# ISAE-PNX/SaDVIO

Measured on AMD Instinct MI355X. Metric: BA iterations/sec (ms/solve in ms_per_solve), 20-KF/8k-landmark window, higher is better.
Workload: dtype f64; 1 GPU; synthetic 20 KF x 8000 landmarks x 40000 reprojection factors (pixel), GN 10 iters (LM step attempts, early exits disabled); windows_per_gpu=1, parallelism=single window, n_kf=20, n_lmk=8000, n_obs=40000, reduced_dim=114

## Files before the change

### sadvio_amd/csrc/ba_capi.hip

```cpp
#include <hip/hip_runtime.h>
#include <dlfcn.h>

#include <algorithm>
#include <chrono>
#include <cmath>
#include <cstdio>
#include <cstdlib>
#include <cstring>
#include <map>
#include <string>
#include <vector>

#include "../../include/sadvio_ba.h"
#include "kernels.h"
#include "dense_chol.h"
#include "marg_kernels.h"
#include "lm_kernels.h"
#include "viinit_kernels.h"
#include "nofov_kernels.h"

using namespace sadvio;

namespace {

// ... 161 lines not shown
struct TriLevel { int first, count, max_m, max_n; };
struct MargScratch {
    DevBuf<double> A, b, G, V, ev, Vs, Ainv, T, Ak, bk, newJ, newr, lastJ, lastr, L, Tb, Zt, S, mi, jsel, lam, wtmp, Hl;
    DevBuf<int> ditems, flag, sel, lastcol, piv_of, lc, piv_mm;
    DevBuf<MargSmall> small;
    DevBuf<NfrSpecC> spec;
    std::vector<int> lcol, items, items_l, col;
    std::vector<double> hev, hS;
    struct TriPlan { DevBuf<TriNode> nodes; std::vector<TriLevel> levels; int leaves = 0; };
    std::map<int, TriPlan> tri_plans;
};

struct LineSetHost {
    std::vector<int64_t> id;
    std::vector<double> T, model, meas;
    std::vector<unsigned char> is_const;
    std::vector<int> ptr, obs_kf, obs_cam;
    int n() const { return (int)id.size(); }
};

struct LayoutScratch {
    std::vector<double> kf_T0, kf_vel, kf_ba, kf_bg, cam_K, cam_T, cam_isig, lmk_p, obs_meas;
    std::vector<int> kf_fidx, lmk_ob, lmk_oe, obs_kf, obs_cam, tile_kf, tile_row, pkf, pcam, run_max, idx, mark, add, kfs, slot_of, chunk_ob, chunk_lm, perm;
    std::vector<unsigned char> lmk_const, obs_slot, obs_lslot;
    std::vector<char> held;
};

struct EnvCfg {
    int debug = 0;
    int lm = -1, pf_wg = -1;
    int tile_rounds = 0, lm_subs = 0, band_c = 0;
    double jacobi_tol = 1e-14;
    bool marg_last_small = false, marg_eig_mm = false, marg_pivoted = false, marg_unpivoted = false, pchol_swap = false, pchol_strict = false,
         jacobi_b4 = false, jacobi_plain = false, no_lpt = false, no_pre = false, no_fork = false, no_bcr = false, imu_items = false;
    void read() {
        auto on = [](const char* k) { return getenv(k) != nullptr; };
        auto num = [](const char* k, int unset) { const char* e = getenv(k); return e ? atoi(e) : unset; };
        debug = num("SADVIO_DEBUG", 0); lm = num("SADVIO_LM", -1); pf_wg = num("SADVIO_PF_WG", -1);
        tile_rounds = num("SADVIO_TILE_ROUNDS", 0); lm_subs = num("SADVIO_LM_SUBS", 0); band_c = num("SADVIO_BAND_C", 0);
        if (const char* e = getenv("SADVIO_JACOBI_TOL")) jacobi_tol = atof(e);
        marg_last_small = on("SADVIO_MARG_LAST_SMALL"); marg_eig_mm = on("SADVIO_MARG_EIG_MM"); marg_pivoted = on("SADVIO_MARG_PIVOTED");
        marg_unpivoted = on("SADVIO_MARG_UNPIVOTED"); pchol_swap = on("SADVIO_PCHOL_SWAP"); pchol_strict = on("SADVIO_PCHOL_STRICT");
        jacobi_b4 = on("SADVIO_JACOBI_B4"); jacobi_plain = on("SADVIO_JACOBI_PLAIN"); no_lpt = on("SADVIO_NO_LPT"); no_pre = on("SADVIO_NO_PRE"); no_fork = on("SADVIO_NO_FORK");
        no_bcr = on("SADVIO_NO_BCR");
        imu_items = on("SADVIO_IMU_ITEMS");
    }
};

struct sadvio_ba_handle {
    EnvCfg env;
    sadvio_ba_config cfg{};
    LayoutScratch ls;
    int device = 0;
    hipStream_t stream = nullptr;
    std::string err;
    std::vector<HostWin> wins;
    std::vector<Tile> tiles;
    std::vector<PriorDev> priors;
    std::vector<int> obs_perm;
    std::vector<std::vector<PriorDev>> priors_per_win;
    std::vector<std::vector<ImuDev>> imus_per_win;
    std::vector<ImuDev> imus;
    int n_kf_tot = 0, n_cam_tot = 0, n_lmk_tot = 0, n_obs_tot = 0, np_tot = 0;
    long long s_tot = 0;
    int factor_type = 0;
    int max_n_kf = 0, max_npose = 0, max_np = 0, n_big = 0;
    DevBuf<int> d_big_info;
    DevBuf<double> d_big_M;
    DevBuf<double> d_big_Lx;
    DevBuf<double> d_big_linv;
    DevBuf<double> d_coll_band;
    DevBuf<double> d_bcr;
    DevBuf<double> d_big_mid;
    bool uploaded = false, solved = false;
    bool defer = false, pending = false;
    UploadBatch up;
// ... 8 lines not shown
    MargScratch mg;
    std::vector<SrcWin> src;
    std::vector<std::vector<char>> sp_elim;
    std::vector<int> n_obs_user;
    std::vector<std::vector<sadvio_sparse_prior>> sparse_per_win;
    std::vector<LineSetHost> lines_per_win;
    DevBuf<LineDev> d_lines;
    DevBuf<LineObsDev> d_lobs;
    DevBuf<double> d_xline, d_line_scratch;
    int n_line_tot = 0, n_lobs_tot = 0;
    DevBuf<SparseDev> d_sparse;
    DevBuf<int> d_sp_list;
    int n_sp_list = 0;
    size_t n_sparse_tot = 0;
    DevBuf<double> d_sp_scratch;
    std::vector<unsigned char> h_lmk_const_user;
    std::vector<int> h_lmk_ob, h_lmk_oe, h_kf_fidx, h_obs_kf;
    bool user_lmk_const = false;
    int n_kept = 0;
    DevBuf<int> d_lmk_red, d_kept_obs, d_dp_ints;
    DevBuf<double> d_dp_data;
    int slots_cap = 0;
    int last_slots = 0;
    DevBuf<WinDev> d_win;
    DevBuf<Tile> d_tiles;
    DevBuf<double> d_kf_T0, d_xp, d_xv, d_xba, d_xbg, d_kf_vel, d_kf_ba, d_kf_bg;
    DevBuf<int> d_kf_fidx;
    DevBuf<double> d_cam_K, d_cam_T, d_cam_isig;
    DevBuf<double> d_lmk_p, d_xl, d_s_lmk;
    DevBuf<unsigned char> d_lmk_const;
    DevBuf<int> d_lmk_ob, d_lmk_oe, d_obs_kf, d_obs_cam, d_tile_kf, d_tile_row;
    DevBuf<int> d_pre_lane, d_pre_kf;
    bool pre_ok = false, pre_dirty = false;
    DevBuf<int> d_rank_col; DevBuf<double> d_rank_x;
    DevBuf<unsigned char> d_obs_slot, d_obs_lslot;
    DevBuf<int> d_chunk_ob, d_chunk_lm, d_tile_perm;
    DevBuf<int> d_jac_ints;
    DevBuf<double> d_jac_dbl;
    DevBuf<double> d_lm_hg, d_lm_dt, d_lm_sacc;
    DevBuf<int> d_lm_sub;
    int lm_n_sub = 0, lm_ksub = 1, lm_sub_per_item = 8;
    int lm_max_cam = 1;
    int hidden_eig_count = 0;
    int marg_stats[4] = {0, 0, 0, 0};
    int lm_sub_obs = 0;
    bool gemm_run4 = false;
    bool lm_ok = false;
    long long lm_landmarks = 0;
    DevBuf<double> d_ptab;
    int max_tile_kf = 1, max_tile_free = 0, max_gemm_free = 0;
    DevBuf<double> d_obs_meas;
    DevBuf<PriorDev> d_priors;
    DevBuf<double> d_prior_lin;
    DevBuf<ImuDev> d_imus;
    DevBuf<double> d_imu_scratch;
    DevBuf<double> d_S, d_gred, d_gfull, d_hdiag, d_delta, d_s_pose;
    DevBuf<LmState> d_states;
    DevBuf<double> d_trace;
    DevBuf<long long> d_tstart;
    DevBuf<IterAcc> d_acc;
    DevBuf<FinalRec> d_final;
    FinalRec* h_final = nullptr;
    double* h_deltas = nullptr; size_t h_deltas_cap = 0; bool deltas_cached = false;
    size_t h_final_n = 0;
    std::vector<FinalRec> fin;
    DevBuf<TileAcc> d_tacc;
// ... 35 lines not shown
        (void)hipEventRecord(h->ev_pool[pool].first, h->stream);
    }
    ~ScopedTimer() {
        if (pool >= 0) (void)hipEventRecord(h->ev_pool[pool].second, h->stream);
    }
};

void collect_timers(sadvio_ba_handle* h) {
    for (auto& u : h->ev_used) {
        float ms = 0;
        if (hipEventElapsedTime(&ms, h->ev_pool[u.second].first, h->ev_pool[u.second].second) == hipSuccess) {
            h->kclasses[u.first].total_ms += ms;
            h->kclasses[u.first].launches += 1;
        }
    }
    h->ev_used.clear();
    h->ev_next = 0;
}

DevPtrs make_ptrs(sadvio_ba_handle* h, const SolveOpts& o, int state_stride) {
    DevPtrs P{};
    P.win = h->d_win.p; P.tiles = h->d_tiles.p;
    P.kf_T0 = h->d_kf_T0.p; P.kf_fidx = h->d_kf_fidx.p;
    P.xp = h->d_xp.p; P.xv = h->d_xv.p; P.xba = h->d_xba.p; P.xbg = h->d_xbg.p;
    P.xp_stride = 6LL * h->n_kf_tot; P.xv_stride = 3LL * h->n_kf_tot; P.xl_stride = 3LL * h->n_lmk_tot;
    P.kf_vel = h->d_kf_vel.p; P.kf_ba = h->d_kf_ba.p; P.kf_bg = h->d_kf_bg.p;
    P.cam_K = h->d_cam_K.p; P.cam_T = h->d_cam_T.p; P.cam_isig = h->d_cam_isig.p;
    P.lmk_p = h->d_lmk_p.p; P.xl = h->d_xl.p; P.s_lmk = h->d_s_lmk.p;
    P.lmk_const = h->has_lmk_const ? h->d_lmk_const.p : nullptr;
    P.lmk_ob = h->d_lmk_ob.p; P.lmk_oe = h->d_lmk_oe.p;
    P.obs_kf = h->d_obs_kf.p; P.obs_cam = h->d_obs_cam.p; P.obs_meas = h->d_obs_meas.p;
    P.obs_slot = h->d_obs_slot.p; P.tile_kf = h->d_tile_kf.p; P.tile_row = h->d_tile_row.p;
    P.pre_lane = h->pre_ok ? (const int4*)h->d_pre_lane.p : nullptr; P.pre_kf = h->pre_ok ? (const int2*)h->d_pre_kf.p : nullptr;
    P.ptab = h->d_ptab.p; P.ptab_stride = (long long)POSE_TAB * h->n_kf_tot;
    P.priors = h->d_priors.p; P.prior_lin = h->d_prior_lin.p; P.prior_lin_stride = (long long)h->priors.size() * PRIOR_LIN; P.n_prior_tot = (int)h->priors.size();
    P.imus = h->d_imus.p; P.imu_scratch = h->d_imu_scratch.p; P.imu_scratch_stride = (long long)h->imus.size() * IMU_ROW;
    P.S = h->d_S.p; P.gred = h->d_gred.p; P.gfull = h->d_gfull.p; P.hdiag = h->d_hdiag.p;
    P.delta = h->d_delta.p; P.s_pose = h->d_s_pose.p;
    P.dbg_ts = h->d_dbg.p;
    P.trace = h->d_trace.p; P.t_start = h->d_tstart.p;
    P.states = h->d_states.p; P.acc = h->d_acc.p; P.tacc = h->d_tacc.p; P.n_tiles = (int)h->tiles.size();
    P.state_stride = state_stride;
    P.final_out = h->h_final ? h->h_final : h->d_final.p;
    P.big_info = h->d_big_info.p;
    P.world = h->world; P.rank = h->rank; P.rank_b = h->d_rank_b.p; P.rank_s = h->d_rank_s.p;
    P.lmk_red = h->d_lmk_red.p; P.kept_obs = h->d_kept_obs.p; P.n_kept = h->n_kept;
    P.dp_data = h->d_dp_data.p; P.dp_ints = h->d_dp_ints.p;
    P.sparse = h->d_sparse.p; P.sp_scratch = h->d_sp_scratch.p; P.sp_list = h->d_sp_list.p;
    P.sp_scratch_stride = (long long)std::max<size_t>(h->n_sparse_tot, 1) * SPARSE_J; P.n_imu_tot = (int)h->imus.size(); P.n_sp_list = h->n_sp_list;
    P.chunk_ob = h->d_chunk_ob.p; P.chunk_lm = h->d_chunk_lm.p; P.tile_perm = h->d_tile_perm.p; P.obs_lslot = h->d_obs_lslot.p;
    P.lm_hg = h->d_lm_hg.p; P.lm_hg_stride = (long long)LM_HG * std::max(h->n_lmk_tot, 1);
    P.lm_dt = h->d_lm_dt.p; P.lm_dt_stride = (long long)LM_DT * std::max<long long>((long long)h->tiles.size(), 1) * h->lm_ksub;
    P.lm_sub = h->d_lm_sub.p; P.lm_ksub = h->lm_ksub; P.lm_sub_per_item = h->lm_sub_per_item; P.lm_sacc = h->lm_ok ? h->d_lm_sacc.p : nullptr;
    P.lines = h->d_lines.p; P.lobs = h->d_lobs.p; P.xline = h->d_xline.p; P.line_scratch = h->d_line_scratch.p;
    P.xline_stride = 6LL * h->n_line_tot;
    P.n_xp = (long long)h->d_xp.n; P.n_xv = (long long)h->d_xv.n; P.n_xl = (long long)h->d_xl.n;
    P.n_win = (int)h->wins.size();
    P.debug = h->env.debug;
    P.o = o;
    return P;
}

__global__ void k_dense_prior_prepare(const double* J, double* Jt, int nf, int n) {
    const long long idx = (long long)blockIdx.x * blockDim.x + threadIdx.x;
    if (idx < (long long)nf * n) {
        const int i = (int)(idx / n), a = (int)(idx - (long long)i * n);
// ... 705 lines not shown
        h->up.add(h->d_lm_sub.p, sub.data(), sub.size() * sizeof(int));
    }
    if (h->env.debug) {
        int hist[32] = {0}, modes[3] = {0};
        for (auto& t : h->tiles) { hist[std::min(t.n_free, 31)]++; modes[t.lds_mode]++; }
        fprintf(stderr, "[sadvio dbg] %zu tiles, modes global/atomic/gemm = %d/%d/%d, max_tile_kf %d, n_free histogram:", h->tiles.size(), modes[0], modes[1], modes[2], h->max_tile_kf);
        for (int i = 0; i < 32; i++) if (hist[i]) fprintf(stderr, " %d:%d", i, hist[i]);
        fprintf(stderr, "\n");
    }
    HIP_TRY(h->d_win.alloc(n_windows)); HIP_TRY(h->d_tacc.alloc(2 * h->tiles.size()));
    if (tile_kf.empty()) { tile_kf.push_back(0); tile_row.push_back(-1); }
    HIP_TRY(h->d_tile_kf.alloc(tile_kf.size())); HIP_TRY(h->d_tile_row.alloc(tile_row.size()));
    HIP_TRY(h->d_obs_slot.alloc(obs_slot.size())); HIP_TRY(h->d_ptab.alloc(2 * (size_t)POSE_TAB * kf_b));
    HIP_TRY(h->d_kf_T0.alloc(kf_T0.size())); HIP_TRY(h->d_kf_fidx.alloc(kf_fidx.size()));
    HIP_TRY(h->d_xp.alloc(2 * 6 * (size_t)kf_b)); HIP_TRY(h->d_xv.alloc(2 * 3 * (size_t)kf_b));
    HIP_TRY(h->d_xba.alloc(2 * 3 * (size_t)kf_b)); HIP_TRY(h->d_xbg.alloc(2 * 3 * (size_t)kf_b));
    HIP_TRY(h->d_kf_vel.alloc(kf_vel.size())); HIP_TRY(h->d_kf_ba.alloc(kf_ba.size())); HIP_TRY(h->d_kf_bg.alloc(kf_bg.size()));
    HIP_TRY(h->d_cam_K.alloc(cam_K.size())); HIP_TRY(h->d_cam_T.alloc(cam_T.size())); HIP_TRY(h->d_cam_isig.alloc(cam_isig.size()));
    HIP_TRY(h->d_lmk_p.alloc(lmk_p.size())); HIP_TRY(h->d_xl.alloc(2 * 3 * (size_t)std::max(lmk_b, 1)));
    HIP_TRY(h->d_s_lmk.alloc(3 * (size_t)std::max(lmk_b, 1)));
    HIP_TRY(h->d_lmk_ob.alloc(lmk_ob.size())); HIP_TRY(h->d_lmk_oe.alloc(lmk_oe.size()));
    HIP_TRY(h->d_obs_kf.alloc(obs_kf.size())); HIP_TRY(h->d_obs_cam.alloc(obs_cam.size())); HIP_TRY(h->d_obs_meas.alloc(obs_meas.size()));
#define UP(dst, src) h->up.add((dst).p, (src).data(), (src).size() * sizeof((src)[0]))
    UP(h->d_kf_T0, kf_T0); UP(h->d_kf_fidx, kf_fidx); UP(h->d_kf_vel, kf_vel);
    UP(h->d_kf_ba, kf_ba); UP(h->d_kf_bg, kf_bg); UP(h->d_cam_K, cam_K); UP(h->d_cam_T, cam_T); UP(h->d_cam_isig, cam_isig);
    if (lmk_b) { UP(h->d_lmk_p, lmk_p); }
    UP(h->d_lmk_ob, lmk_ob); UP(h->d_lmk_oe, lmk_oe); UP(h->d_obs_kf, obs_kf);
    UP(h->d_obs_cam, obs_cam); UP(h->d_obs_meas, obs_meas); UP(h->d_tile_kf, tile_kf); UP(h->d_tile_row, tile_row); UP(h->d_obs_slot, obs_slot);
    h->pre_ok = !h->tiles.empty() && h->tiles.size() <= PRE_MAX_TILES && !h->env.no_pre;
    if (h->pre_ok) {
        HIP_TRY(h->d_pre_lane.alloc((size_t)4 * (BUILD_THREADS / 8) * h->tiles.size())); HIP_TRY(h->d_pre_kf.alloc((size_t)2 * PRE_KF * h->tiles.size()));
        h->pre_dirty = true;
    }
#undef UP
    h->h_lmk_const_user = lmk_const; h->user_lmk_const = h->has_lmk_const;
    h->h_lmk_ob = lmk_ob; h->h_lmk_oe = lmk_oe; h->h_kf_fidx = kf_fidx; h->h_obs_kf = obs_kf;
    lap("alloc+queue");
    int rc = layout_reduced(h);
    if (rc != SADVIO_OK) return rc;
    lap("layout_reduced");
    rc = upload_priors(h);
    if (rc != SADVIO_OK) return rc;
    lap("flush");
    h->uploaded = true;
    for (auto& k : h->kclasses) { k.total_ms = 0; k.launches = 0; }
    return SADVIO_OK;
}

int sadvio_ba_set_windows(sadvio_ba_handle* h, int32_t n_windows, const sadvio_flat_window* wins) {
    if (!h) return SADVIO_E_INVALID_ARG;
    if (n_windows <= 0 || !wins) { h->err = "set_windows: no windows"; return SADVIO_E_INVALID_ARG; }
    h->uploaded = false; h->solved = false;
    for (int w = 0; w < n_windows; w++) {
        const sadvio_flat_window& F = wins[w];
        if (F.n_kf <= 0 || F.n_cam < 0 || F.n_lmk < 0 || F.n_obs < 0 || !F.kf_T_f_w || (F.n_cam > 0 && (!F.cam_K || !F.cam_T_s_f)) ||
            (F.n_obs > 0 && F.n_cam == 0) ||
            (F.n_lmk > 0 && (!F.lmk_p || !F.lmk_obs_ptr)) || (F.n_obs > 0 && (!F.obs_kf || !F.obs_cam || !F.obs_meas))) {
            h->err = "set_windows: missing array in window " + std::to_string(w);
            return SADVIO_E_INVALID_ARG;
        }
        if (F.n_lmk > 0 && (F.lmk_obs_ptr[0] != 0 || F.lmk_obs_ptr[F.n_lmk] != F.n_obs)) {
            h->err = "set_windows: lmk_obs_ptr is not a CSR over n_obs";
            return SADVIO_E_INVALID_ARG;
        }
        for (int l = 0; l < F.n_lmk; l++)
            if (F.lmk_obs_ptr[l + 1] < F.lmk_obs_ptr[l]) { h->err = "set_windows: CSR not monotone"; return SADVIO_E_INVALID_ARG; }
// ... 1517 lines not shown
        h->max_gemm_free = 0;
        Rp = 0; strip_doubles = STAGE_VALS * 64;
        lds_build = tile_tables_bytes(mtk) + sizeof(double) * ((size_t)BUILD_WAVES * strip_doubles + nt * (nt + 1) / 2 + 3 * nt +
                                                               0) + 16;
    }
    if (h->env.debug) fprintf(stderr, "[sadvio dbg] lds_build %zu B, Rp %d, strip_doubles %d, max_tile_kf %d, max_tile_free %d, tiles %d\n", lds_build, Rp, strip_doubles, mtk, h->max_tile_free, n_tiles);
    const size_t lds_back = tile_tables_bytes(mtk) + sizeof(double) * ((size_t)mtk * 18) + 16;
    const size_t npq = (size_t)h->max_np;
    const size_t lds_solve = sizeof(double) * ((size_t)c16_size((int)npq) + 4 * npq + 1 + C16_WORK + 16 * (size_t)c16_blocks((int)npq + 1) + SOLVE_KFC * SOLVE_KFC_STRIDE) + 64;
    bool any_pseudo = false;
    for (const auto& v : h->sp_elim) for (char e : v) any_pseudo |= e != 0;
    bool any_kept_lmk = false;
    for (int w = 0; w < n_win; w++) any_kept_lmk |= h->wins[w].d.n_red > 0;
    const bool rare = o.huber_a > 0.0 || h->n_kept > 0 || any_kept_lmk || any_pseudo || h->gemm_run4;
    const bool pix = h->factor_type == SADVIO_FACTOR_PIXEL;
    const bool have_pf = !h->imus.empty() || h->n_sp_list > 0;
    bool with_imu = have_pf && n_tiles <= 3 * 256;
    if (h->env.pf_wg >= 0) with_imu = have_pf && h->env.pf_wg != 0;
    auto kb = with_imu ? (pix ? (rare ? k_build<0, true, true> : k_build<0, false, true>) : (rare ? k_build<1, true, true> : k_build<1, false, true>))
                       : (pix ? (rare ? k_build<0, true, false> : k_build<0, false, false>) : (rare ? k_build<1, true, false> : k_build<1, false, false>));
    auto kk = with_imu ? (pix ? (rare ? k_backsub<0, true, true> : k_backsub<0, false, true>) : (rare ? k_backsub<1, true, true> : k_backsub<1, false, true>))
                       : (pix ? (rare ? k_backsub<0, true, false> : k_backsub<0, false, false>) : (rare ? k_backsub<1, true, false> : k_backsub<1, false, false>));
    auto kbk = h->factor_type == SADVIO_FACTOR_PIXEL ? k_build_kept<0> : k_build_kept<1>;
    bool use_lm = h->lm_ok && !rare && !h->coll_fn && h->world == 1 && h->lm_landmarks >= 65536;
    if (h->env.lm >= 0) use_lm = h->lm_ok && !rare && !h->coll_fn && h->world == 1 && h->env.lm != 0;
    auto kbo = pix ? k_build_obs<0> : k_build_obs<1>;
    auto kps = pix ? k_lm_pass<0, false> : k_lm_pass<1, false>;
    auto kps0 = pix ? k_lm_pass<0, true> : k_lm_pass<1, true>;
    const size_t lds_views = pix ? sizeof(double) * (size_t)mtk * h->lm_max_cam * LM_VT : 0;
    const size_t lds_bobs = tile_tables_bytes(mtk) + sizeof(double) * ((size_t)BUILD_WAVES * Rp * LM_KS + nt * (nt + 1) / 2 + nt + 1 + LM_DT) + lds_views + 16;
    const size_t lds_pass0 = tile_tables_bytes(mtk) + sizeof(double) * LM_DT_COST + (size_t)h->lm_sub_obs * ((pix ? 2 : 3) * sizeof(double) + sizeof(int)) + lds_views + 16;
    const size_t lds_pass = lds_pass0 + sizeof(double) * (size_t)mtk * (POSE_TAB + 6) + lds_views;
    if (!use_lm) P.lm_sacc = nullptr;
    if (use_lm) {
        P.decide_kernel = 1;
        HIP_TRY(hipFuncSetAttribute((const void*)kbo, hipFuncAttributeMaxDynamicSharedMemorySize, (int)lds_bobs));
        HIP_TRY(hipFuncSetAttribute((const void*)kps, hipFuncAttributeMaxDynamicSharedMemorySize, (int)lds_pass));
        HIP_TRY(hipFuncSetAttribute((const void*)kps0, hipFuncAttributeMaxDynamicSharedMemorySize, (int)lds_pass0));
    }
    HIP_TRY(hipFuncSetAttribute((const void*)kb, hipFuncAttributeMaxDynamicSharedMemorySize, (int)lds_build));
    HIP_TRY(hipFuncSetAttribute((const void*)kk, hipFuncAttributeMaxDynamicSharedMemorySize, (int)lds_back));
    bool extras = false;
    for (int w = 0; w < n_win; w++) {
        const WinDev& d = h->wins[w].d;
        if (d.imu_end > d.imu_begin || d.sp_end > d.sp_begin || d.dp_n_full > 0 || d.dpf == 15 || d.lobs_end > d.lobs_begin || d.line_end > d.line_begin) extras = true;
    }
    auto ks0 = extras ? k_solve<0, true> : k_solve<0, false>;
    auto ks1 = extras ? k_solve<1, true> : k_solve<1, false>;
    auto ks2 = extras ? k_solve<2, true> : k_solve<2, false>;
    HIP_TRY(hipFuncSetAttribute((const void*)ks0, hipFuncAttributeMaxDynamicSharedMemorySize, (int)lds_solve));
    const int reset_blocks = (int)std::min<long long>(1024, std::max<long long>(1, (P.n_xl + P.n_xp + 255) / 256));
    std::vector<BigPlan> big(n_win);
    for (int w = 0; w < n_win; w++) {
        const WinDev& d = h->wins[w].d;
        if (!d.ld) continue;
        int hb = h->wins[w].hb_lmk;
        for (const ImuDev& f : h->imus_per_win[w]) {
            const int fi = h->h_kf_fidx[f.kf_i], fj = h->h_kf_fidx[f.kf_j];
            if (fi >= 0 && fj >= 0) hb = std::max(hb, std::abs(fi - fj));
        }
        if (w < (int)h->sparse_per_win.size())
            for (const sadvio_sparse_prior& sp : h->sparse_per_win[w])
                if (sp.type == SADVIO_SPARSE_RELATIVE_POSE) {
                    const int fi = h->h_kf_fidx[d.kf_base + sp.kf], fj = h->h_kf_fidx[d.kf_base + sp.kf_b];
                    if (fi >= 0 && fj >= 0) hb = std::max(hb, std::abs(fi - fj));
                }
// ... 103 lines not shown
            if (fork) {
                (void)hipEventRecord(h->ev_solved, h->stream);
                (void)hipStreamWaitEvent(h->side, h->ev_solved, 0);
                if (n_lo) hipLaunchKernelGGL(k_line_eval<false>, dim3(n_lo), dim3(64), 0, h->side, P, s, 0);
                (void)hipEventRecord(h->ev_cost, h->side);
            } else {
                if (n_lo) { ScopedTimer t(h, "k_line_cost"); hipLaunchKernelGGL(k_line_eval<false>, dim3(n_lo), dim3(64), 0, h->stream, P, s, 0); }
            }
            if (dp_max_nf > 0) { ScopedTimer t(h, "k_prior_m"); hipLaunchKernelGGL(k_prior_m, dim3((dp_max_nf + 3) / 4, n_win), dim3(256), 0, h->stream, P, s); }
            if (n_pf && (use_lm || !with_imu)) { ScopedTimer t(h, "k_pf_cost"); hipLaunchKernelGGL(k_pf_eval<true>, dim3(n_pf), dim3(64), 0, h->stream, P, s); }
            if (use_lm) {
                ScopedTimer t(h, "k_lm_pass"); hipLaunchKernelGGL(kps, dim3(h->lm_n_sub), dim3(LM_PASS_THREADS), lds_pass, h->stream, P, s, mtk, h->lm_sub_obs);
            }
            else
            { ScopedTimer t(h, "k_backsub"); hipLaunchKernelGGL(kk, dim3(n_tiles + (with_imu ? n_pf : 0)), dim3(BUILD_THREADS), lds_back, h->stream, P, s, mtk); }
            if (fork) (void)hipStreamWaitEvent(h->stream, h->ev_cost, 0);
            if (h->coll_fn) {
                { ScopedTimer t(h, "k_rank_partials"); hipLaunchKernelGGL(k_rank_partials, dim3(n_win), dim3(64), 0, h->stream, P, s, 1); }
                ScopedTimer t(h, "allreduce_step_partials");
                if (h->coll_fn(h->coll_ctx, h->d_rank_s.p, (int64_t)n_win * h->world * 4, (void*)h->stream) != 0) coll_failed = true;
            }
            if (P.decide_kernel) { ScopedTimer t(h, "k_decide"); hipLaunchKernelGGL(k_decide, dim3(n_win), dim3(max_win_tiles > 4 * BUILD_THREADS ? 1024 : 64), 0, h->stream, P, s, 0); }
        }
        { ScopedTimer t(h, "k_final"); hipLaunchKernelGGL(k_decide, dim3(n_win), dim3(64), 0, h->stream, P, slots - 1, 1); }
    };
    if (h->cfg.use_graph && !h->cfg.profile_kernels && !h->coll_fn) {
        std::vector<int> lay;
        for (int w = 0; w < n_win; w++) { lay.push_back(h->wins[w].d.Np); lay.push_back(h->wins[w].d.ld); lay.push_back(big[w].bw); }
        lay.push_back(h->n_kept); lay.push_back(h->lm_sub_obs); lay.push_back(h->lm_n_sub); lay.push_back(h->lm_max_cam); lay.push_back(h->n_lobs_tot); lay.push_back(h->n_line_tot); lay.push_back(h->n_big); lay.push_back(dp_max_nf); lay.push_back(dp_max_n);
        std::vector<unsigned char> key(sizeof(DevPtrs) + 8 * sizeof(int) + 3 * sizeof(size_t) + lay.size() * sizeof(int));
        unsigned char* kp = key.data();
        memcpy(kp + sizeof(DevPtrs) + 8 * sizeof(int) + 3 * sizeof(size_t), lay.data(), lay.size() * sizeof(int));
        memcpy(kp, &P, sizeof(DevPtrs)); kp += sizeof(DevPtrs);
        const int env_bits = (int)with_imu + 2 * (int)h->env.no_fork + 32 * (int)h->env.no_bcr + 128 * (int)h->env.no_lpt;
        const int ints[8] = {slots, n_tiles, n_win, mtk, strip_doubles, Rp, h->n_kf_tot, h->factor_type + 2 * (int)extras + 4 * (int)rare + 8 * (int)use_lm + 16 * env_bits};
        memcpy(kp, ints, sizeof(ints)); kp += sizeof(ints);
        const size_t szs[3] = {lds_build, lds_back, lds_solve};
        memcpy(kp, szs, sizeof(szs));
        if (!h->graph_exec || key != h->graph_key) {
            if (h->graph_exec) { (void)hipGraphExecDestroy(h->graph_exec); h->graph_exec = nullptr; }
            hipGraph_t g = nullptr;
            HIP_TRY(hipStreamBeginCapture(h->stream, hipStreamCaptureModeThreadLocal));
            enqueue();
            HIP_TRY(hipStreamEndCapture(h->stream, &g));
            HIP_TRY(hipGraphInstantiate(&h->graph_exec, g, nullptr, nullptr, 0));
            (void)hipGraphDestroy(g);
            h->graph_key = key;
        }
        HIP_TRY(hipGraphLaunch(h->graph_exec, h->stream));
    } else {
        enqueue();
    }
    HIP_TRY(hipGetLastError());
    if (coll_failed) { h->err = "solve: the all-reduce of the reduced system failed"; return SADVIO_E_RCCL; }
    HIP_TRY(hipStreamSynchronize(h->stream));
    if (h->cfg.profile_kernels) collect_timers(h);
    if ((h->env.debug & 4096)) {
        long long ts[128];
        if (hipMemcpy(ts, h->d_dbg.p, sizeof(ts), hipMemcpyDeviceToHost) == hipSuccess) {
            fprintf(stderr, "[sadvio dbg] phase dt (us):");
            for (int i = 1; i < 16; i++) fprintf(stderr, " %d:%.2f", i, (ts[i] - ts[0]) * 0.01);
            fprintf(stderr, "  shader clock %.3f GHz\n[sadvio dbg] k_build:", (double)(ts[21] - ts[20]) / ((ts[15] - ts[0]) * 10.0));
            for (int i = 33; i < 43; i++) fprintf(stderr, " %d:%.2f", i, (ts[i] - ts[32]) * 0.01);
            fprintf(stderr, "\n[sadvio dbg] first IMU pair of k_build, us since its start (residual + Jacobian on lane 0 | decision | W J | entries + adds): %.2f %.2f %.2f %.2f, start %.2f us after tile 0",
                    (ts[57] - ts[56]) * 0.01, (ts[58] - ts[56]) * 0.01, (ts[59] - ts[56]) * 0.01, (ts[60] - ts[56]) * 0.01, (ts[56] - ts[32]) * 0.01);
            fprintf(stderr, "\n[sadvio dbg] k_wchol_step (panel 1), us since the workgroup's start: look-ahead (operands in LDS | substituted | block updated | factored) %.2f %.2f %.2f %.2f",
                    (ts[107] - ts[106]) * 0.01, (ts[108] - ts[106]) * 0.01, (ts[109] - ts[106]) * 0.01, (ts[110] - ts[106]) * 0.01);
// ... 394 lines not shown
```

### sadvio_amd/csrc/ba_types.h

```cpp
#pragma once
#include <stdint.h>

namespace sadvio {

struct SolveOpts {
    int max_num_iterations;
    int jacobi_scaling;
    int max_num_consecutive_invalid_steps;
    int pad;
    double function_tolerance, gradient_tolerance, parameter_tolerance;
    double initial_radius, max_radius, min_radius;
    double min_lm_diagonal, max_lm_diagonal, min_relative_decrease;
    double huber_a;
    double max_time_ticks;
};

struct WinDev {
    int n_kf, n_cam, n_lmk, n_obs;
    int kf_base, cam_base, lmk_base, obs_base;
    int n_free_kf, dpf, Np, Npose;
    long long S_off;
    int red_off;
    int tile_begin, tile_end;
    int prior_begin, prior_end;
// ... 88 lines not shown

struct IterAcc {
    double lin_cost;
    double cand_cost;
    double mcc;
    double step_norm2;
    double cand_norm2;
    double fixed_cost;
    unsigned long long gmax_bits;
    int chol_fail;
    int time_up;
};

struct TileAcc {
    double lin_cost, fixed_cost, gmax;
    double cand_cost, mcc, step_norm2, cand_norm2;
    double pad;
};

constexpr int BUILD_THREADS = 256;
constexpr int BUILD_WAVES = BUILD_THREADS / 64;
constexpr int MAX_TILE_KF = 24;
constexpr int MAX_TILE_FREE_KF = 20;
constexpr int MAX_GEMM_FREE_KF = 5;
constexpr int MAX_WIN_CAM = 8;
constexpr int STAGE_VALS = 18;
constexpr int MAX_LMK_OBS = 64;
constexpr int SOLVE_THREADS = 512;
constexpr int SOLVE_KFC_STRIDE = 32;
constexpr int SOLVE_KFC = 32;
constexpr int PRIOR_LIN = 28;
constexpr int PRE_KF = 8;
constexpr int PRE_MAX_TILES = 1024;
constexpr int MAX_LDS_NP = 174;

}
```

### sadvio_amd/csrc/kernels.h

```cpp
#pragma once
#include "ba_types.h"
#include "device_math.h"
#include "chol16.h"

namespace sadvio {

struct DevPtrs {
    const WinDev* win;
    const Tile* tiles;
    const double* kf_T0;
    const int* kf_fidx;
    double* xp; double* xv; double* xba; double* xbg;
    long long xp_stride, xv_stride, xl_stride;
    const double* kf_vel; const double* kf_ba; const double* kf_bg;
    const double* cam_K; const double* cam_T; const double* cam_isig;
    const double* lmk_p; double* xl; double* s_lmk;
    const unsigned char* lmk_const;
    const int* lmk_ob; const int* lmk_oe;
    const int* obs_kf; const int* obs_cam; const double* obs_meas;
    const unsigned char* obs_slot;
    const int* tile_kf;
    const int* tile_row;
    const int4* pre_lane;
    const int2* pre_kf;
    double* ptab;
    long long ptab_stride;
    const PriorDev* priors;
    double* prior_lin;
    long long prior_lin_stride;
    int n_prior_tot;
    const ImuDev* imus;
    double* imu_scratch;
    long long imu_scratch_stride;
    double* S; double* gred; double* gfull; double* hdiag; double* delta; double* s_pose;
    LmState* states;
    IterAcc* acc;
    TileAcc* tacc;
    FinalRec* final_out;
    int* big_info;
    int imu_direct;
    int decide_kernel;
    int world, rank;
    double* rank_b;
    double* rank_s;
    const int* lmk_red;
    const int* kept_obs;
    int n_kept;
    double* dp_data;
    const SparseDev* sparse;
    const int* sp_list;
    double* sp_scratch;
    long long sp_scratch_stride;
    int n_imu_tot, n_sp_list;
    const int* dp_ints;
    const int* chunk_ob;
    const int* chunk_lm;
    const int* tile_perm;
// ... 544 lines not shown
        const int nobs = lmk_valid ? oe - ob : 0;
        const int lcode = first ? pre_lcode : (P.lmk_const ? P.lmk_const[gl] : 0);
        const bool lfree = lcode == 0;
        ObsLin L;
        L.valid = q < nobs;
        L.row = -1; L.slot = 0; L.counted = false;
        if (L.valid) {
            double pw[3];
            ObsPre obq;
            if (first) {
#pragma unroll
                for (int i = 0; i < 3; i++) pw[i] = pre_p[i] + (st.cur ? pre_x1[i] : pre_x0[i]);
                obq = pre_obs;
            } else {
#pragma unroll
                for (int i = 0; i < 3; i++) pw[i] = P.lmk_p[3 * (long long)gl + i] + xl[3 * (long long)gl + i];
                obq = obs_prefetch<FACTOR>(P, ob + q);
            }
            lane_linearize<FACTOR, RARE>(P, poseTab, camTab, rowTab, T.cam_base, obq, pw, lfree, lcode != 1, L);
            const double c = L.rho;
            if (L.counted) cost_part += c;
            else { fixed_part += c; L.r[0] = 0.0; L.r[1] = 0.0; }
        } else {
            L.r[0] = L.r[1] = 0.0;
#pragma unroll
            for (int i = 0; i < 12; i++) L.Jp[i] = 0.0;
#pragma unroll
            for (int i = 0; i < 6; i++) L.Jl[i] = 0.0;
        }
    SADVIO_TS(3, 35);
        double Mi[6], g[3];
        const bool active = group_eliminate(P, L, G, gl, lmk_valid, lfree, nobs, st.radius, slot == 0, q == 0, Mi, g);
        if (active && q == 0) gmax_part = fmax(gmax_part, fmax(fabs(g[0]), fmax(fabs(g[1]), fabs(g[2]))));
    SADVIO_TS(3, 36);
        double N[6], gam[3];
        li_row(Mi, L.Jl[0], L.Jl[1], L.Jl[2], N);
        li_row(Mi, L.Jl[3], L.Jl[4], L.Jl[5], N + 3);
        li_vec(Mi, g, gam);
        if (gemm_mode) {
            constexpr int Kw = 32, KS = Kw + 2;
            double* Yb = wstage;
            const double* Eb = Yb;
            {
                double2* z = (double2*)wstage;
                const double2 zero2 = make_double2(0.0, 0.0);
                for (int i = ln; i < Rp * KS / 2; i += 64) z[i] = zero2;
            }
            const bool vrow = L.valid && L.row >= 0;
            const int myrow = vrow ? L.row : -2 - ln;
            const int row_prev = dpp_i32<0x111>(myrow);
            const int row_next = dpp_i32<0x101>(myrow);
            const bool follower = vrow && q > 0 && row_prev == myrow;
            const bool has_follower = vrow && q + 1 < G && row_next == myrow;
            const int row_next2 = RARE ? dpp_i32<0x102>(myrow) : -1;
            const bool has_follower2 = RARE && vrow && q + 2 < G && row_next2 == myrow;
            const bool head = vrow && !follower;
            const double rt0 = L.r[0] - (N[0] * gam[0] + N[1] * gam[1] + N[2] * gam[2]);
            const double rt1 = L.r[1] - (N[3] * gam[0] + N[4] * gam[1] + N[5] * gam[2]);
            wave_lds_fence();
    SADVIO_TS(3, 37);
#pragma unroll
            for (int i = 0; i < 6; i++) {
                const double j0 = vrow ? L.Jp[i] : 0.0, j1 = vrow ? L.Jp[6 + i] : 0.0;
                double y[3];
#pragma unroll
                for (int c = 0; c < 3; c++) {
// ... 1105 lines not shown
        acc->step_norm2 = a0; acc->cand_norm2 = a1; acc->mcc = a2; acc->cand_cost = a3;
    }
    SADVIO_TS(3, 8);
    if (ts && tid == 0) { ts[15] = wall_clock64(); ts[21] = clock64(); }
}


__device__ __forceinline__ void zero_s_slice(const DevPtrs& P, const Tile& T, int tile_index) {
    if (T.ld != 0) return;
    const int n2 = c16_size(T.Np) >> 1;
    const int per = (n2 + T.win_ntiles - 1) / T.win_ntiles;
    const int i0 = (tile_index - T.win_tile0) * per, i1 = min(i0 + per, n2);
    double2* S2 = (double2*)(P.S + T.S_off);
    const double2 z2 = make_double2(0.0, 0.0);
    for (int i = i0 + (int)threadIdx.x; i < i1; i += blockDim.x) S2[i] = z2;
}

template <int FACTOR, bool RARE, bool IMU>
__global__ __launch_bounds__(BUILD_THREADS) void k_backsub(DevPtrs P, int slot, int max_tile_kf) {
    extern __shared__ __attribute__((aligned(16))) char smem[];
    if (IMU && (int)blockIdx.x >= P.n_tiles) {
        if (threadIdx.x < 64) pose_factor_eval<true>(P, slot, (int)blockIdx.x - P.n_tiles, threadIdx.x);
        return;
    }
    const Tile T = P.tiles[blockIdx.x];
    const int tid = threadIdx.x, wv = tid >> 6, ln = tid & 63;
    int4 pl = make_int4(0, -1, 0, 0);
    int2 pk = make_int2(-1, -1), pk6 = make_int2(-1, -1);
    if (P.pre_lane) {
        pl = P.pre_lane[(long long)blockIdx.x * (BUILD_THREADS / 8) + (tid >> 3)];
        pk = P.pre_kf[(long long)blockIdx.x * PRE_KF + tid / POSE_TAB];
        if (tid < PRE_KF * 6) pk6 = P.pre_kf[(long long)blockIdx.x * PRE_KF + tid / 6];
    }
    LmState st;
    int chol_fail;
    if (P.n_win == 1) { st = P.states[slot]; chol_fail = P.acc[slot].chol_fail; }
    else { st = P.states[(long long)T.w * P.state_stride + slot]; chol_fail = P.acc[(long long)T.w * P.state_stride + slot].chol_fail; }
    zero_s_slice(P, T, blockIdx.x);
    double* poseTab = (double*)smem;
    double* camTab = poseTab + (size_t)max_tile_kf * POSE_TAB;
    int* rowTab = (int*)(camTab + MAX_WIN_CAM * 17);
    double* candTab = (double*)(smem + tile_tables_bytes(max_tile_kf));
    double* dpTab = candTab + (size_t)max_tile_kf * 12;
    const int G = T.G, lpw = 64 / G;
    const int grp = ln / G, q = ln - grp * G;
    const int nl = T.lmk1 - T.lmk0;
    bool first_valid;
    int gl_first, pre_ob, pre_oe, pre_o;
    if (P.pre_lane) {
        first_valid = (pl.z >> 16) & 1; gl_first = pl.x; pre_ob = pl.y; pre_oe = pl.y + (pl.z & 0xff);
        pre_o = (pl.w + (tid & 7) < (pl.z & 0xff)) ? pl.y + pl.w + (tid & 7) : -1;
    } else {
        first_valid = wv * lpw + grp < nl;
        gl_first = T.lmk0 + (first_valid ? wv * lpw + grp : 0);
        pre_ob = P.lmk_ob[gl_first]; pre_oe = P.lmk_oe[gl_first];
        pre_o = (first_valid && q < pre_oe - pre_ob) ? pre_ob + q : -1;
    }
    const int pre_lcode = P.lmk_const ? P.lmk_const[gl_first] : 0;
    double pre_p[3], pre_xa[3], pre_xb[3];
#pragma unroll
    for (int i = 0; i < 3; i++) {
        pre_p[i] = P.lmk_p[3 * (long long)gl_first + i];
        pre_xa[i] = P.xl[3 * (long long)gl_first + i];
        pre_xb[i] = P.xl[P.xl_stride + 3 * (long long)gl_first + i];
    }
    ObsPre pre_obs;
// ... 62 lines not shown
    double sn = 0.0, cn = 0.0, mcc = 0.0, cc = 0.0;
    for (int base = wv * lpw; base < nl; base += BUILD_WAVES * lpw) {
        const int lm = base + grp;
        const bool lmk_valid = lm < nl;
        const int gl = T.lmk0 + (lmk_valid ? lm : 0);
        const bool first = base == wv * lpw;
        const int ob = first ? pre_ob : P.lmk_ob[gl], oe = first ? pre_oe : P.lmk_oe[gl];
        const int nobs = lmk_valid ? oe - ob : 0;
        const int lcode = first ? pre_lcode : (P.lmk_const ? P.lmk_const[gl] : 0);
        const bool lfree = lcode == 0;
        double p0[3], x0[3];
#pragma unroll
        for (int i = 0; i < 3; i++) {
            p0[i] = first ? pre_p[i] : P.lmk_p[3 * (long long)gl + i];
            x0[i] = first ? pre_x[i] : xl[3 * (long long)gl + i];
        }
        ObsLin L;
        L.valid = q < nobs;
        L.row = -1; L.slot = 0; L.counted = false;
        ObsPre obq = pre_obs;
        if (L.valid) {
            const double pw[3] = {p0[0] + x0[0], p0[1] + x0[1], p0[2] + x0[2]};
            if (!first) obq = obs_prefetch<FACTOR>(P, ob + q);
            lane_linearize<FACTOR, RARE>(P, poseTab, camTab, rowTab, T.cam_base, obq, pw, lcode != 1, lcode != 1, L);
            if (!L.counted) { L.r[0] = 0.0; L.r[1] = 0.0; }
        } else {
            L.r[0] = L.r[1] = 0.0;
#pragma unroll
            for (int i = 0; i < 12; i++) L.Jp[i] = 0.0;
#pragma unroll
            for (int i = 0; i < 6; i++) L.Jl[i] = 0.0;
        }
        double Mi[6], g[3];
        const bool active = group_eliminate(P, L, G, gl, lmk_valid, lfree, nobs, st.radius, false, false, Mi, g);

        double e0 = L.r[0], e1 = L.r[1];
        const double* d = dpTab + L.slot * 6;
        if (L.valid && L.row >= 0) {
#pragma unroll
            for (int i = 0; i < 6; i++) { e0 += L.Jp[i] * d[i]; e1 += L.Jp[6 + i] * d[i]; }
        }
        const double tt[3] = {group_sum(L.Jl[0] * e0 + L.Jl[3] * e1, G), group_sum(L.Jl[1] * e0 + L.Jl[4] * e1, G),
                              group_sum(L.Jl[2] * e0 + L.Jl[5] * e1, G)};
        double ut[3], vt3[3];
        li_vec(Mi, tt, ut);
        li_tvec(Mi, ut, vt3);
        double d0 = -vt3[0], d1 = -vt3[1], d2 = -vt3[2];
        if (RARE && lcode == 2) {
            const double* dr = P.delta + T.red_off + P.lmk_red[gl];
            d0 = dr[0]; d1 = dr[1]; d2 = dr[2];
        }
        const double c0 = x0[0] + d0, c1 = x0[1] + d1, c2 = x0[2] + d2;
        if (lmk_valid && q == 0) {
            xlc[3 * (long long)gl] = c0; xlc[3 * (long long)gl + 1] = c1; xlc[3 * (long long)gl + 2] = c2;
            if (active) {
                sn += d0 * d0 + d1 * d1 + d2 * d2;
                cn += c0 * c0 + c1 * c1 + c2 * c2;
            } else if (RARE && lcode == 2 && (P.world == 1 || P.rank == 0)) cn += c0 * c0 + c1 * c1 + c2 * c2;
        }
        if (L.valid && L.counted) {
            const double m0 = (e0 - L.r[0]) + L.Jl[0] * d0 + L.Jl[1] * d1 + L.Jl[2] * d2;
            const double m1 = (e1 - L.r[1]) + L.Jl[3] * d0 + L.Jl[4] * d1 + L.Jl[5] * d2;
            mcc += -m0 * (L.r[0] + 0.5 * m0) - m1 * (L.r[1] + 0.5 * m1);
            const int craw = obq.craw;
            const int cam = craw < 0 ? 0 : craw - T.cam_base;
            const double* ct = camTab + cam * 17;
            const double pw[3] = {p0[0] + c0, p0[1] + c1, p0[2] + c2};
// ... 952 lines not shown
```

Before: 18020 BA iterations/s.

## Record per-landmark Schur inverse factors in build and reuse them in backsub

The build kernel now writes each landmark's 6-value inverse factor (Mi) from group elimination to a per-tile global record buffer, using nontemporal stores. The backsubstitution kernel reads these values back per lane instead of re-running group_eliminate, which skips redundant 3x3 accumulation, reductions and factorisation work. The path is enabled only when precomputed lanes exist, tiles fit in a single pass, and the solve is neither LM nor rare, and it can be disabled with an environment variable. In exchange it adds global memory traffic, a new buffer, and a dependency on lane mapping consistency between the two kernels.

```diff
diff --git a/sadvio_amd/csrc/ba_capi.hip b/sadvio_amd/csrc/ba_capi.hip
--- a/sadvio_amd/csrc/ba_capi.hip
+++ b/sadvio_amd/csrc/ba_capi.hip
@@ -217,7 +217,7 @@
     int tile_rounds = 0, lm_subs = 0, band_c = 0;
     double jacobi_tol = 1e-14;
     bool marg_last_small = false, marg_eig_mm = false, marg_pivoted = false, marg_unpivoted = false, pchol_swap = false, pchol_strict = false,
-         jacobi_b4 = false, jacobi_plain = false, no_lpt = false, no_pre = false, no_fork = false, no_bcr = false, imu_items = false;
+         jacobi_b4 = false, jacobi_plain = false, no_lpt = false, no_pre = false, no_rec = false, no_fork = false, no_bcr = false, imu_items = false;
     void read() {
         auto on = [](const char* k) { return getenv(k) != nullptr; };
         auto num = [](const char* k, int unset) { const char* e = getenv(k); return e ? atoi(e) : unset; };
@@ -226,7 +226,7 @@
         if (const char* e = getenv("SADVIO_JACOBI_TOL")) jacobi_tol = atof(e);
         marg_last_small = on("SADVIO_MARG_LAST_SMALL"); marg_eig_mm = on("SADVIO_MARG_EIG_MM"); marg_pivoted = on("SADVIO_MARG_PIVOTED");
         marg_unpivoted = on("SADVIO_MARG_UNPIVOTED"); pchol_swap = on("SADVIO_PCHOL_SWAP"); pchol_strict = on("SADVIO_PCHOL_STRICT");
-        jacobi_b4 = on("SADVIO_JACOBI_B4"); jacobi_plain = on("SADVIO_JACOBI_PLAIN"); no_lpt = on("SADVIO_NO_LPT"); no_pre = on("SADVIO_NO_PRE"); no_fork = on("SADVIO_NO_FORK");
+        jacobi_b4 = on("SADVIO_JACOBI_B4"); jacobi_plain = on("SADVIO_JACOBI_PLAIN"); no_lpt = on("SADVIO_NO_LPT"); no_pre = on("SADVIO_NO_PRE"); no_rec = on("SADVIO_NO_REC"); no_fork = on("SADVIO_NO_FORK");
         no_bcr = on("SADVIO_NO_BCR");
         imu_items = on("SADVIO_IMU_ITEMS");
     }
@@ -301,6 +301,8 @@
     DevBuf<int> d_lmk_ob, d_lmk_oe, d_obs_kf, d_obs_cam, d_tile_kf, d_tile_row;
     DevBuf<int> d_pre_lane, d_pre_kf;
     bool pre_ok = false, pre_dirty = false;
+    DevBuf<double> d_step_rec;
+    bool rec_ok = false;
     DevBuf<int> d_rank_col; DevBuf<double> d_rank_x;
     DevBuf<unsigned char> d_obs_slot, d_obs_lslot;
     DevBuf<int> d_chunk_ob, d_chunk_lm, d_tile_perm;
@@ -402,6 +404,7 @@
     P.obs_kf = h->d_obs_kf.p; P.obs_cam = h->d_obs_cam.p; P.obs_meas = h->d_obs_meas.p;
     P.obs_slot = h->d_obs_slot.p; P.tile_kf = h->d_tile_kf.p; P.tile_row = h->d_tile_row.p;
     P.pre_lane = h->pre_ok ? (const int4*)h->d_pre_lane.p : nullptr; P.pre_kf = h->pre_ok ? (const int2*)h->d_pre_kf.p : nullptr;
+    P.step_rec = h->rec_ok ? h->d_step_rec.p : nullptr;
     P.ptab = h->d_ptab.p; P.ptab_stride = (long long)POSE_TAB * h->n_kf_tot;
     P.priors = h->d_priors.p; P.prior_lin = h->d_prior_lin.p; P.prior_lin_stride = (long long)h->priors.size() * PRIOR_LIN; P.n_prior_tot = (int)h->priors.size();
     P.imus = h->d_imus.p; P.imu_scratch = h->d_imu_scratch.p; P.imu_scratch_stride = (long long)h->imus.size() * IMU_ROW;
@@ -1173,6 +1176,10 @@
         HIP_TRY(h->d_pre_lane.alloc((size_t)4 * (BUILD_THREADS / 8) * h->tiles.size())); HIP_TRY(h->d_pre_kf.alloc((size_t)2 * PRE_KF * h->tiles.size()));
         h->pre_dirty = true;
     }
+    h->rec_ok = h->pre_ok && !h->env.no_rec;
+    for (const Tile& t : h->tiles) if (t.lmk1 - t.lmk0 > BUILD_WAVES * (64 / t.G)) h->rec_ok = false;
+    if (h->rec_ok) HIP_TRY(h->d_step_rec.alloc((size_t)REC_NF * BUILD_THREADS * h->tiles.size()));
+    else h->d_step_rec.release();
 #undef UP
     h->h_lmk_const_user = lmk_const; h->user_lmk_const = h->has_lmk_const;
     h->h_lmk_ob = lmk_ob; h->h_lmk_oe = lmk_oe; h->h_kf_fidx = kf_fidx; h->h_obs_kf = obs_kf;
@@ -2756,6 +2763,7 @@
     const size_t lds_pass0 = tile_tables_bytes(mtk) + sizeof(double) * LM_DT_COST + (size_t)h->lm_sub_obs * ((pix ? 2 : 3) * sizeof(double) + sizeof(int)) + lds_views + 16;
     const size_t lds_pass = lds_pass0 + sizeof(double) * (size_t)mtk * (POSE_TAB + 6) + lds_views;
     if (!use_lm) P.lm_sacc = nullptr;
+    if (rare || use_lm) P.step_rec = nullptr;
     if (use_lm) {
         P.decide_kernel = 1;
         HIP_TRY(hipFuncSetAttribute((const void*)kbo, hipFuncAttributeMaxDynamicSharedMemorySize, (int)lds_bobs));
@@ -2925,7 +2933,7 @@
         unsigned char* kp = key.data();
         memcpy(kp + sizeof(DevPtrs) + 8 * sizeof(int) + 3 * sizeof(size_t), lay.data(), lay.size() * sizeof(int));
         memcpy(kp, &P, sizeof(DevPtrs)); kp += sizeof(DevPtrs);
-        const int env_bits = (int)with_imu + 2 * (int)h->env.no_fork + 32 * (int)h->env.no_bcr + 128 * (int)h->env.no_lpt;
+        const int env_bits = (int)with_imu + 2 * (int)h->env.no_fork + 32 * (int)h->env.no_bcr + 128 * (int)h->env.no_lpt + 256 * (int)h->env.no_rec;
         const int ints[8] = {slots, n_tiles, n_win, mtk, strip_doubles, Rp, h->n_kf_tot, h->factor_type + 2 * (int)extras + 4 * (int)rare + 8 * (int)use_lm + 16 * env_bits};
         memcpy(kp, ints, sizeof(ints)); kp += sizeof(ints);
         const size_t szs[3] = {lds_build, lds_back, lds_solve};
diff --git a/sadvio_amd/csrc/ba_types.h b/sadvio_amd/csrc/ba_types.h
--- a/sadvio_amd/csrc/ba_types.h
+++ b/sadvio_amd/csrc/ba_types.h
@@ -144,6 +144,7 @@
 constexpr int PRIOR_LIN = 28;
 constexpr int PRE_KF = 8;
 constexpr int PRE_MAX_TILES = 1024;
+constexpr int REC_NF = 6;
 constexpr int MAX_LDS_NP = 174;
 
 }
diff --git a/sadvio_amd/csrc/kernels.h b/sadvio_amd/csrc/kernels.h
--- a/sadvio_amd/csrc/kernels.h
+++ b/sadvio_amd/csrc/kernels.h
@@ -23,6 +23,7 @@
     const int* tile_row;
     const int4* pre_lane;
     const int2* pre_kf;
+    double* step_rec;
     double* ptab;
     long long ptab_stride;
     const PriorDev* priors;
@@ -633,6 +634,11 @@
         double Mi[6], g[3];
         const bool active = group_eliminate(P, L, G, gl, lmk_valid, lfree, nobs, st.radius, slot == 0, q == 0, Mi, g);
         if (active && q == 0) gmax_part = fmax(gmax_part, fmax(fabs(g[0]), fmax(fabs(g[1]), fabs(g[2]))));
+        if (!RARE && P.step_rec && L.valid && q == 0) {
+            double* rec = P.step_rec + (long long)blockIdx.x * (REC_NF * BUILD_THREADS) + tid;
+#pragma unroll
+            for (int i = 0; i < REC_NF; i++) __builtin_nontemporal_store(Mi[i], rec + i * BUILD_THREADS);
+        }
     SADVIO_TS(3, 36);
         double N[6], gam[3];
         li_row(Mi, L.Jl[0], L.Jl[1], L.Jl[2], N);
@@ -1804,6 +1810,15 @@
         pk = P.pre_kf[(long long)blockIdx.x * PRE_KF + tid / POSE_TAB];
         if (tid < PRE_KF * 6) pk6 = P.pre_kf[(long long)blockIdx.x * PRE_KF + tid / 6];
     }
+    const bool use_rec = !RARE && P.step_rec != nullptr;
+    double rc[REC_NF];
+#pragma unroll
+    for (int f = 0; f < REC_NF; f++) rc[f] = 0.0;
+    if (use_rec && ((pl.z >> 16) & 1) && (pl.z & 0xff) > 0) {
+        const double* rec = P.step_rec + (long long)blockIdx.x * (REC_NF * BUILD_THREADS) + (tid - (pl.w + (tid & 7)));
+#pragma unroll
+        for (int f = 0; f < REC_NF; f++) rc[f] = rec[f * BUILD_THREADS];
+    }
     LmState st;
     int chol_fail;
     if (P.n_win == 1) { st = P.states[slot]; chol_fail = P.acc[slot].chol_fail; }
@@ -1932,7 +1947,12 @@
             for (int i = 0; i < 6; i++) L.Jl[i] = 0.0;
         }
         double Mi[6], g[3];
-        const bool active = group_eliminate(P, L, G, gl, lmk_valid, lfree, nobs, st.radius, false, false, Mi, g);
+        bool active;
+        if (use_rec) {
+#pragma unroll
+            for (int i = 0; i < 6; i++) Mi[i] = L.valid ? rc[i] : 0.0;
+            active = lmk_valid && lfree && nobs > 0;
+        } else active = group_eliminate(P, L, G, gl, lmk_valid, lfree, nobs, st.radius, false, false, Mi, g);
 
         double e0 = L.r[0], e1 = L.r[1];
         const double* d = dpTab + L.slot * 6;
```

New measurement: 18210 BA iterations/s (median of 6 runs). 1.01x the previous value.
